# elybrand/quantized_neural_networks

Hardware: AMD Instinct MI355X
Metric: weights_quantized_per_sec (higher is better)
Workload: dtype f64; 1 GPU; Dense(4096->4096) whole-layer GPFQ, m=1024 calibration samples, M=3 alphabet, alphabet_scalar=3 (BASELINE.json configs[1], the north-star layer); N=4096, C=4096, m=1024, M=3, neurons_per_gpu=4096, arithmetic=f32 products / f64 residual and dot products (reference's mixed flow)

## Files before the change

quantized_neural_networks_amd/csrc/gpfq_blk.hip:

```cpp
#include <atomic>
#include <cmath>
#include <cstring>
#include <type_traits>

#include <cstdlib>
#include <mutex>
#include "gpfq_device.hpp"
#include <hip/hip_ext.h>
#include "gpfq_launch.hpp"
#include "gpfq_roles.hpp"

namespace gpfq {

namespace {

struct BlkStats {
    double rden, G, cb, ca, Ea, nrm;
    double sE1, sE2;
};
struct BandEntry {
    double H1, H2, E1, E2;
};
static_assert(sizeof(BlkStats) == 64 && sizeof(BandEntry) == 32, "header layout");

// ... 234 lines not shown
            for (int d = ND - 1; d >= 1; --d) { wx[d] = wx[d - 1]; wq[d] = wq[d - 1]; }
            wx[0] = xc; wq[0] = qc4;
            xc = xc1; qc4 = qc1; qn = qn1;
        }
    }
    __syncthreads();
    for (int w = threadIdx.x; w < RUN * (ND + 1); w += 256) {
        const int r = w / (ND + 1), e = w - r * (ND + 1);
        const int64_t t = t0 + r;
        if (t >= nrec) continue;
        auto total = [&](int k) { return (sm[r][0][k] + sm[r][1][k]) + (sm[r][2][k] + sm[r][3][k]); };
        char *rb = recs + t * rbytes;
        if (e == 0) {
            BlkStats st{};
            const double nrm = t < N ? (own_norms ? (double)(float)sqrt(nsm[r][0] + nsm[r][1] + nsm[r][2] + nsm[r][3]) : (double)nrm32[t]) : 0.0;
            const double s1 = total(1), s2 = total(2);
            st.nrm = nrm;
            st.rden = nrm < 1e-16 ? 0.0 : 1.0 / (nrm * nrm);
            st.G = total(0);
            st.cb = 0x1p-23 * s1 * st.rden * up;
            st.ca = 0x1p-149 * s2 * st.rden * up;
            st.Ea = 0x1p-149 * s2 * up;
            double e1 = 0.0, e2 = 0.0;
#pragma unroll
            for (int d = 1; d <= ND; ++d) { e1 += total(5 + 4 * (d - 1)); e2 += total(6 + 4 * (d - 1)); }
            st.sE1 = 0x1p-23 * e1 * up * up; st.sE2 = 0x1p-23 * e2 * up * up;
            *reinterpret_cast<BlkStats *>(rb) = st;
            *reinterpret_cast<BlkStats *>(hdrs + t * hdr) = st;
        } else {
            const int d = e;
            BandEntry be;
            be.H1 = total(3 + 4 * (d - 1)); be.H2 = total(4 + 4 * (d - 1));
            be.E1 = 0x1p-23 * total(5 + 4 * (d - 1)) * up; be.E2 = 0x1p-23 * total(6 + 4 * (d - 1)) * up;
            *reinterpret_cast<BandEntry *>(rb + 64 + 32 * (d - 1)) = be;
            *reinterpret_cast<BandEntry *>(hdrs + t * hdr + 64 + 32 * (d - 1)) = be;
        }
    }
}

__global__ void __launch_bounds__(256)
gpfq_blk_scale_kernel(char *__restrict__ recs, int64_t rec_bytes, int hdr, int mps, int64_t slice_bytes, const DevAlphabet *__restrict__ alpha)
{
    const float a = alpha->sym_a;
    float4 *row = reinterpret_cast<float4 *>(recs + (int64_t)blockIdx.y * slice_bytes + (int64_t)blockIdx.x * rec_bytes + hdr + 4 * (int64_t)mps);
    for (int i = threadIdx.x; i < mps / 4; i += 256) {
        const float4 v = row[i];
        row[i] = make_float4(__fmul_rn(a, v.x), __fmul_rn(a, v.y), __fmul_rn(a, v.z), __fmul_rn(a, v.w));
    }
}

template <int G, int NL, bool CL = false> constexpr bool blk_sweep_flush() { return (G == 4 && NL == 1) || CL; }

struct BlkLds {
    int tile_bytes, tile_pitch, off_w, off_d, off_wq, off_x2, off_e, off_out, off_ctl, off_zero, off_hr, hr_pitch, total;
};
constexpr int kOutSteps = 32;

__host__ __device__ constexpr int blk_sublanes(int nb) { return 64 / nb > 8 ? 8 : 64 / nb; }
__host__ __device__ constexpr int blk_slots(int nsw, int nb) { return (nsw + blk_sublanes(nb) - 1) / blk_sublanes(nb) * blk_sublanes(nb); }

__host__ __device__ inline BlkLds blk_lds(int mp, int nb, int B, int nsw, int G, bool CL = false)
{
    BlkLds L;
    const int nw = blk_slots(nsw, nb);
    L.tile_bytes = B * (int)blk_rec_bytes(mp, B, G, CL);
    L.tile_pitch = (L.tile_bytes + 1023) & ~1023;
    int o = 2 * L.tile_pitch;
    L.off_w = o;    o += 2 * nb * B * 4;    o = (o + 15) & ~15;
    L.off_d = o;    o += 2 * nw * B * nb * 8;
    L.off_wq = o;   o += 2 * nb * B * 8;
    L.off_x2 = o;   o += nw * nb * 16;
    L.off_e = o;    o += 68 * 8;
    L.off_out = o;  o += nb * kOutSteps * 8;
    L.off_ctl = o;  o += 16;
    L.off_zero = o; o += 32;
    o = (o + 15) & ~15;
    L.hr_pitch = (B * blk_hdr_bytes(B, CL) + 1023) & ~1023;
    L.off_hr = o;   o += 3 * L.hr_pitch;
    L.total = o;
    return L;
}

struct BlkK {
    const char *recs;
    const char *hdrs;
    const float *Wt;
    int64_t ldw, ldt;
    int64_t N, C;
    int m, M, zero_idx, nblk;
    int8_t *qidx;
    float *Qt;
    int64_t o_sj, o_st;
    const DevAlphabet *alpha;
    int *alpha_err;
    double *resid, *u_out;
    unsigned long long *fallback_count;
    unsigned long long *stamps;
    const float *Xq;
    int64_t ldx;
    unsigned char pw[12];
    int nsl;
    int cl_map;
    int64_t slice_bytes;
    unsigned long long *mbox;
    int64_t u_ld;
    double slack;
    int *cl_err;
    unsigned long long cl_timeout;
    int cl_fault;
};

#ifdef GPFQ_BLK_DIAG
#include "gpfq_blk_diag.hpp"
#else
constexpr bool kNoMfmaD = false, kNoFused = false;
#define STAMP(var) do { } while (0)
#define STAMP_DO(...)
#endif

struct ClState { int64_t cl; int slice; unsigned seq; bool dead; int64_t rec_off; int m_sl; };
typedef unsigned cl_u32x4 __attribute__((ext_vector_type(4)));

__device__ __forceinline__ cl_u32x4 cl_load16(const unsigned long long *p)
{
    cl_u32x4 r;
    asm volatile("global_load_dwordx4 %0, %1, off sc1" : "=&v"(r) : "v"(p) : "memory");
    return r;
}

template <int KV>
__device__ __forceinline__ void cl_publish(const BlkK &K, ClState &cs, int lane, const double (&v)[KV])
{
    const unsigned seq = ++cs.seq;
    if (K.cl_fault && cs.cl == 0 && cs.slice == 1) return;
    unsigned long long *buf = K.mbox + ((cs.cl * 2 + (int64_t)(seq & 1u)) * (int64_t)K.nsl) * 256;
    unsigned long long *mine = buf + ((int64_t)cs.slice * 64 + lane) * 4;
#pragma unroll
    for (int k = 0; k < KV; ++k) {
        const cl_u32x4 w = {(unsigned)__double2loint(v[k]), seq, (unsigned)__double2hiint(v[k]), seq};
        asm volatile("global_store_dwordx4 %0, %1, off sc1" :: "v"(mine + 2 * k), "v"(w) : "memory");
    }
}

template <int KV, int CLB>
__device__ __forceinline__ void cl_gather(const BlkK &K, ClState &cs, int lane, double (&v)[KV])
{
    const unsigned seq = cs.seq;
    const unsigned long long *buf = K.mbox + ((cs.cl * 2 + (int64_t)(seq & 1u)) * (int64_t)K.nsl) * 256;
    double tot[KV];
#pragma unroll
    for (int k = 0; k < KV; ++k) tot[k] = 0.0;
    const unsigned long long t0 = __builtin_amdgcn_s_memrealtime();
    for (int s0 = 0; s0 < K.nsl; s0 += CLB) {
        cl_u32x4 w[CLB][KV];
        for (;;) {
#pragma unroll
            for (int i = 0; i < CLB; ++i) {
                const unsigned long long *p = buf + ((int64_t)(s0 + i < K.nsl ? s0 + i : cs.slice) * 64 + lane) * 4;
#pragma unroll
                for (int k = 0; k < KV; ++k) w[i][k] = cl_load16(p + 2 * k);
            }
            asm volatile("s_waitcnt vmcnt(0)" ::: "memory");
// ... 166 lines not shown
        for (;;) {
            const int S = __builtin_amdgcn_readfirstlane(ctl);
            if (S < 0) break;
            const int nb_ = ((b + 1) & 1) * L.tile_pitch;
            const int cbq = (b & 1) * NB * B * 8;
            double eu[NL], ew[NL];
#pragma unroll
            for (int n = 0; n < NL; ++n) { eu[n] = 0.0; ew[n] = 0.0; }
#pragma unroll
            for (int n = 0; n < NL; ++n) {
                const float w = lds_ld<float2>(lds, o_wq + cbq + (n * B + S) * 8).x;
#pragma unroll 1
                for (int p = 0; p < PW; ++p) {
                    double t0 = u[n][0], t1 = u[n][1];
#pragma unroll
                    for (int pp = 1; pp < PW; ++pp) { t0 = (p == pp) ? u[n][2 * pp] : t0; t1 = (p == pp) ? u[n][2 * pp + 1] : t1; }
                    for (int j = 0; j < S; ++j) {
                        const int rb = nb_ + j * RB;
                        const float2 x2 = lds_ld<float2>(lds, rb + o_x + 8 * p * KQ), q2 = lds_ld<float2>(lds, rb + o_q + 8 * p * KQ);
                        const float2 wq = lds_ld<float2>(lds, o_wq + cbq + (n * B + j) * 8);
                        if constexpr (SYM) {
                            t0 += (double)__fmaf_rn(wq.y, q2.x, __fmul_rn(wq.x, x2.x));
                            t1 += (double)__fmaf_rn(wq.y, q2.y, __fmul_rn(wq.x, x2.y));
                        } else {
                            t0 += (double)__fsub_rn(__fmul_rn(wq.x, x2.x), __fmul_rn(wq.y, q2.x));
                            t1 += (double)__fsub_rn(__fmul_rn(wq.x, x2.y), __fmul_rn(wq.y, q2.y));
                        }
                    }
                    const int rb = nb_ + S * RB;
                    const float2 x2 = lds_ld<float2>(lds, rb + o_x + 8 * p * KQ);
                    float2 q2;
                    if constexpr (SYM) {
                        const int i0 = 2 * (pbase + p * KQ + kq);
                        const float *xr = K.Xq + ((int64_t)b * B + S) * K.ldx + (CL ? (int64_t)cs.slice * MP : (int64_t)0);
                        const int mrow = CL ? cs.m_sl : K.m;
                        q2.x = i0 < mrow ? xr[i0] : 0.f;
                        q2.y = i0 + 1 < mrow ? xr[i0 + 1] : 0.f;
                    } else {
                        q2 = lds_ld<float2>(lds, rb + o_q + 8 * p * KQ);
                    }
                    eu[n] = fma((double)q2.x, t0, eu[n]);
                    eu[n] = fma((double)q2.y, t1, eu[n]);
                    ew[n] = fma((double)q2.x, t0 + (double)__fmul_rn(w, x2.x), ew[n]);
                    ew[n] = fma((double)q2.y, t1 + (double)__fmul_rn(w, x2.y), ew[n]);
                }
            }
            const double vu = fold_klanes_n<G, NL>(eu), vw = fold_klanes_n<G, NL>(ew);
            if (writer) lds_st<double2>(lds, o_x2, make_double2(vu, vw));
            slot_barrier();
            slot_barrier();
            ctl = lds_ld<int>(lds, L.off_ctl + 4 * (b & 1));
        }
    };
    for (int b = 0; b < nslots; ++b) {
        STAMP(st0);
        STAMP_DO(if (b) acc_t += st0 - st5;)
        if (blk_sweep_flush<G, NL, CL>() && b >= 1 && wave == b % NSW && lane < NB * B && (!CL || cs.slice == 0)) {
            const int nn = lane / B, sidx = lane % B;
            const int64_t t = (int64_t)(b - 1) * B + sidx, jn = jbase + nn;
            if (t < N && jn < K.C) {
                const int2 v = lds_ld<int2>(lds, L.off_out + (nn * kOutSteps + (int)(t % kOutSteps)) * 8);
                if (K.qidx) K.qidx[jn * N + t] = (int8_t)v.x;
                if (K.Qt) K.Qt[jn * N + t] = __int_as_float(v.y);
            }
        }
        if (b + 1 < nslots) load_weights(b + 1);
        load_headers(b + 2, hbuf); hbuf = hbuf == 2 ? 0 : hbuf + 1;
        const int bn = b + 1 < nslots ? b + 1 : b;
        STAMP(st1);
        const int tbase = (b & 1) * L.tile_pitch;
        const int pbq = ((b - 1) & 1) * NB * B * 8;

        auto update_pair = [&](int p, const float2 &x2, const float2 &q2, const float (&wv)[NL], const float (&qv)[NL]) {
            const pk2 xv = {x2.x, x2.y}, qx = {q2.x, q2.y};
            pk2 pr[NL], rr[NL], dd[NL];
            double c0[NL], c1[NL];
#pragma unroll
            for (int n = 0; n < NL; ++n) pr[n] = pk2{wv[n], wv[n]} * xv;
            if constexpr (SYM) {
#pragma unroll
                for (int n = 0; n < NL; ++n) dd[n] = __builtin_elementwise_fma(pk2{qv[n], qv[n]}, qx, pr[n]);
            } else {
#pragma unroll
                for (int n = 0; n < NL; ++n) rr[n] = pk2{qv[n], qv[n]} * qx;
#pragma unroll
                for (int n = 0; n < NL; ++n) dd[n] = pr[n] - rr[n];
            }
#pragma unroll
            for (int n = 0; n < NL; ++n) { c0[n] = (double)dd[n].x; c1[n] = (double)dd[n].y; }
#pragma unroll
            for (int n = 0; n < NL; ++n) { u[n][2 * p] += c0[n]; u[n][2 * p + 1] += c1[n]; }
        };
        if constexpr (kFused) {
            const int rbm = tbase + ng * RB + o_d;
            constexpr int PF = NSW == 7 ? 2 : 1, NPS = PW * B;
            float2 fwq[B][NL], xbuf[PF], qbuf[PF];
            double2 dcur;
            auto row_off = [&](int i, bool q) { return tbase + (i % B) * RB + (q ? o_q : o_x) + 8 * (i / B) * KQ; };
            auto first_requests = [&]() {
#pragma unroll
                for (int s = 0; s < B; ++s)
#pragma unroll
                    for (int n = 0; n < NL; ++n) fwq[s][n] = lds_ld<float2>(lds, o_wq + pbq + (n * B + s) * 8);
#pragma unroll
                for (int i = 0; i < PF; ++i)
                    if (i < NPS) { xbuf[i] = lds_ld<float2>(lds, row_off(i, false)); qbuf[i] = lds_ld<float2>(lds, row_off(i, true)); }
                dcur = lds_ld<double2>(lds, rbm);
            };
            first_requests();
            double2 dprev = make_double2(0.0, 0.0);
            double acc[NL];
#pragma unroll
            for (int n = 0; n < NL; ++n) acc[n] = 0.0;
            auto mfma_pair = [&](int pp, int i, const double2 &dd) {
                const int n = i % NL, e = i / NL;
                acc[n] = __builtin_amdgcn_mfma_f64_4x4x4f64(u[n][2 * pp + e], e ? dd.y : dd.x, acc[n], 0, 0, 0);
            };
#pragma unroll
            for (int p = 0; p < PW; ++p) {
                {
                    const int pr = 2 - (3 * p) / PW;
                    if (p == 0 || pr != 2 - (3 * (p - 1)) / PW) {
                        const int v = pr;
                        if (v >= 2) __builtin_amdgcn_s_setprio(2);
                        else if (v == 1) __builtin_amdgcn_s_setprio(1);
                        else __builtin_amdgcn_s_setprio(0);
                    }
                }
                if (p > 0) dcur = lds_ld<double2>(lds, rbm + DB * p * KQ);
#pragma unroll
                for (int st = 0; st < B; ++st) {
                    const int ips = p * B + st;
                    const float2 x2 = xbuf[ips % PF], q2 = qbuf[ips % PF];
                    const int pn = (ips + 1) / B, sn = (ips + 1) % B;
                    (void)pn; (void)sn;
                    if (ips + PF < NPS) {
                        xbuf[ips % PF] = lds_ld<float2>(lds, row_off(ips + PF, false));
                        qbuf[ips % PF] = lds_ld<float2>(lds, row_off(ips + PF, true));
                    }
                    if (p < PTS) {
#pragma unroll
                        for (int i = 0; i < PPP; ++i) {
                            const int k = (PTS * st + p) * PPP + i;
                            if (PTS * B * PPP <= PER_MIN || k < PER_MIN) issue_piece(bn, k);
                        }
                    }
                    __builtin_amdgcn_sched_barrier(0);
                    float wv[NL], qv[NL];
#pragma unroll
                    for (int n = 0; n < NL; ++n) { wv[n] = fwq[st][n].x; qv[n] = fwq[st][n].y; }
                    update_pair(p, x2, q2, wv, qv);
                    if (p > 0) {
#pragma unroll
                        for (int i = 0; i < 2 * NL; ++i)
                            if (i * B / (2 * NL) == st) mfma_pair(p - 1, i, dprev);
                    }
                    __builtin_amdgcn_sched_barrier(0);
                }
                dprev = dcur;
            }
            for (int k = PTS * B * PPP < PER_MIN ? PTS * B * PPP : PER_MIN; wave + NSW * k < NPIECES; ++k) issue_piece(bn, k);
            STAMP(st2);
#pragma unroll
            for (int i = 0; i < 2 * NL; ++i) mfma_pair(PW - 1, i, dprev);
#pragma unroll
            for (int n = 0; n < NL; ++n) { acc[n] = ror_add<8>(acc[n]); acc[n] = ror_add<4>(acc[n]); }
            if (b + 1 < nslots && (lane & 12) == 0) {
                const int od = L.off_d + ((((((b + 1) & 1) * NW + wave) * B) + (lane & 3)) * NB + NL * (lane >> 4)) * 8;
                if constexpr (NL == 4) {
                    lds_st<double2>(lds, od, make_double2(acc[0], acc[1]));
                    lds_st<double2>(lds, od + 16, make_double2(acc[2], acc[3]));
                } else if constexpr (NL == 2) {
                    lds_st<double2>(lds, od, make_double2(acc[0], acc[NL - 1]));
                } else {
                    lds_st<double>(lds, od, acc[0]);
                }
            }
        } else {
        if constexpr (kPreloadAll) {
            if constexpr (!kHoist) { preload_wq(b); preload_rows(b); __builtin_amdgcn_sched_barrier(0); }
#pragma unroll
            for (int s = 0; s < B; ++s) {
                if (s == 0) __builtin_amdgcn_s_setprio(2);
                if (s == B / 2) __builtin_amdgcn_s_setprio(1);
                float wv[NL], qv[NL];
#pragma unroll
                for (int n = 0; n < NL; ++n) { wv[n] = wqa[s][n].x; qv[n] = wqa[s][n].y; }
#pragma unroll
                for (int p = 0; p < PW; ++p) {
                    if (p < PTS) {
#pragma unroll
// ... 78 lines not shown
                for (int p = 0; p < PW; ++p) {
                    if constexpr (kPreD) dsl[r][p] = ds[r][p];
                    else dsl[r][p] = ld_d(tbase + r * RB + o_d + DB * p * KQ);
                }
            if constexpr (!kPreD) __builtin_amdgcn_sched_barrier(0);
#pragma unroll
            for (int r = 0; r < B; ++r) {
                if (r == B / 2) __builtin_amdgcn_s_setprio(0);
                double acc[NL];
#pragma unroll
                for (int n = 0; n < NL; ++n) acc[n] = 0.0;
#pragma unroll
                for (int p = 0; p < PW; ++p) {
                    const double2 d2 = to_d2(dsl[r][p]);
#pragma unroll
                    for (int n = 0; n < NL; ++n) {
                        acc[n] = fma(d2.x, u[n][2 * p], acc[n]);
                        acc[n] = fma(d2.y, u[n][2 * p + 1], acc[n]);
                    }
                }
                const double v = fold_klanes_n<G, NL>(acc);
                if (writer) lds_st<double>(lds, o_dw + ((((b + 1) & 1) * NW) * B + r) * NB * 8, v);
            }
        } else
        if (b + 1 < nslots) {
            DRaw d2n = ld_d(tbase + o_d);
#pragma clang loop unroll_count(B == 4 ? 2 : 1)
            for (int r = 0; r < B; ++r) {
                if (r == B / 2) __builtin_amdgcn_s_setprio(0);
                double acc[NL];
#pragma unroll
                for (int n = 0; n < NL; ++n) acc[n] = 0.0;
                const int rb = tbase + r * RB;
                const int rn = r + 1 < B ? r + 1 : r;
#pragma unroll
                for (int p = 0; p < PW; ++p) {
                    const double2 d2 = to_d2(d2n);
                    const int rbn = p + 1 < PW ? rb : tbase + rn * RB, pn = p + 1 < PW ? p + 1 : 0;
                    d2n = ld_d(rbn + o_d + DB * pn * KQ);
                    __builtin_amdgcn_sched_barrier(0);
#pragma unroll
                    for (int n = 0; n < NL; ++n) {
                        acc[n] = fma(d2.x, u[n][2 * p], acc[n]);
                        acc[n] = fma(d2.y, u[n][2 * p + 1], acc[n]);
                    }
                    __builtin_amdgcn_sched_barrier(0);
                }
                const double v = fold_klanes_n<G, NL>(acc);
                if (writer) lds_st<double>(lds, o_dw + ((((b + 1) & 1) * NW) * B + r) * NB * 8, v);
            }
        }
        }
        STAMP(st3);
        dma_wait();
        STAMP(st4);
        slot_barrier();
        STAMP(st5);
        STAMP_DO(acc_dma += st1 - st0; acc_u += st2 - st1; acc_d += st3 - st2; acc_w += st4 - st3; acc_b += st5 - st4;)

        {
        int ctl = lds_ld<int>(lds, L.off_ctl + 4 * (b & 1));
        if constexpr (kHoist) {
            if (b + 1 < nslots) { preload_wq(b + 1); preload_rows(b + 1); }
        }
        if (__builtin_amdgcn_readfirstlane(ctl) >= 0) {
            slow_path(b, ctl);
            if constexpr (kHoist) {
                if (b + 1 < nslots) { preload_wq(b + 1); preload_rows(b + 1); }
            }
        }
        }
    }

    STAMP_DO(
    if (K.stamps && blockIdx.x == 0 && lane == 0 && (wave == 0 || wave == 7)) {
        unsigned long long *o = K.stamps + (wave == 0 ? 0 : 8);
        o[0] = acc_dma; o[1] = acc_u; o[2] = acc_d; o[3] = acc_w; o[4] = acc_b; o[5] = (unsigned long long)nslots; o[6] = acc_t;
    }
    if (K.stamps && blockIdx.x == 0 && lane == 0) K.stamps[32 + wave] = acc_dma + acc_u + acc_d + acc_w;

    )
    if (K.resid) {
        double ss[NL];
#pragma unroll
        for (int n = 0; n < NL; ++n) {
            double q = 0.0;
#pragma unroll
            for (int e = 0; e < 2 * PW; ++e) q = fma(u[n][e], u[n][e], q);
            ss[n] = q;
        }
        const double v = fold_klanes_n<G, NL>(ss);
        if (writer) lds_st<double>(lds, o_dw, v);
    }
    slot_barrier();
    if (K.u_out) {
#pragma unroll
        for (int n = 0; n < NL; ++n) {
            const int64_t jn = jbase + nloc + n;
            if (jn < K.C) {
#pragma unroll
                for (int p = 0; p < PW; ++p)
#pragma unroll
                    for (int e = 0; e < 2; ++e) {
                        const int i = 2 * (pbase + p * KQ + kq) + e;
                        if constexpr (CL) {
                            if (i < cs.m_sl) K.u_out[jn * K.u_ld + (int64_t)cs.slice * MP + i] = u[n][2 * p + e];
                        } else {
                            if (i < K.m) K.u_out[jn * (int64_t)K.m + i] = u[n][2 * p + e];
                        }
                    }
            }
        }
    }
}

template <int G, int MP, int B, int NSW, bool SYM, int NL, int CLM, bool KOUT = false>
__device__ __forceinline__ void blk_decision_role(const BlkK &K, char *lds_generic, const BlkLds &L, int lane, ClState &cs)
{
    constexpr bool CL = CLM != 0;
    constexpr int NB = NL * G, R = blk_sublanes(NB), NW = blk_slots(NSW, NB);
    constexpr int RB = (int)blk_rec_bytes(MP, B, G, CL);
    lchar *lds = (lchar *)lds_generic;
    const bool shadow = lane / R >= NB;
    const int n = shadow ? NB - 1 : lane / R, r = lane % R;
    const int64_t wg = cs.cl;
    const int64_t jn = wg * NB + n;
    const bool active = jn < K.C;
    const int64_t N = K.N;
    const int M = K.M;
    const int nslots = K.nblk + 1;
    const double kNaN = __longlong_as_double(0x7ff8000000000000LL);
    const int o_d   = L.off_d + (r * B * NB + n) * 8;
    const int o_x2  = L.off_x2 + (r * NB + n) * 16;
    const int o_w   = L.off_w + n * B * 4;
    const int o_wq  = L.off_wq + n * B * 8;
    const int o_out = L.off_out + n * kOutSteps * 8;

    const bool in_regs = M <= 4 * R;

    const double al_a0 = K.alpha->a0, al_step = K.alpha->step, al_inv = K.alpha->inv, al_c0 = K.alpha->c0;
    const unsigned long long al_plus = K.alpha->plus, al_minus = K.alpha->minus;
    const double sym_top = SYM ? lds_ld<double>(lds, L.off_e + 8 * (2 + M - 1)) : 0.0;
    const double sym_hb = (SYM && M == 3) ? 0.5 * sym_top : 0.0;
    float wprev[B], qprev[B];
    float wprev2[B], qprev2[B];
#pragma unroll
    for (int j = 0; j < B; ++j) { wprev[j] = 0.f; qprev[j] = 0.f; wprev2[j] = 0.f; qprev2[j] = 0.f; }
    double DmCur = 0.0;
    (void)wprev2; (void)qprev2; (void)DmCur;
    unsigned long long n_fallback = 0;
    auto wave_min_stop = [&](int v) -> int {
        int mn = B;
#pragma unroll
        for (int k = B - 1; k >= 0; --k)
            if (__ballot(v == k) != 0ull) mn = k;
        return mn;
    };

    constexpr bool kOwnFlush = !blk_sweep_flush<G, NL, CL>();
    auto flush = [&](int64_t t0, int64_t t1) {
        if constexpr (KOUT) {
            constexpr int NJ = NB < 8 ? NB : 8, GJ = NB / NJ;
            for (int e = lane; e < GJ * kOutSteps; e += 64) {
                const int g = e / kOutSteps, c = e % kOutSteps;
                const int64_t ts = t0 + c, j0 = wg * NB + g * NJ;
                if (ts >= t1 || j0 >= K.C || (CL && cs.slice != 0)) continue;
                int idxj[NJ]; float qj[NJ];
#pragma unroll
                for (int k = 0; k < NJ; ++k) {
                    const int2 v = lds_ld<int2>(lds, L.off_out + ((g * NJ + k) * kOutSteps + (int)(ts % kOutSteps)) * 8);
                    idxj[k] = v.x; qj[k] = __int_as_float(v.y);
                }
                const int64_t o = ts * K.o_st + j0;
                const bool whole = j0 + NJ <= K.C && K.o_sj == 1;
                if (K.qidx) {
                    if (whole && NJ >= 4 && ((uintptr_t)(K.qidx + o) & (NJ - 1)) == 0) {
                        unsigned lo = 0, hi = 0;
#pragma unroll
                        for (int k = 0; k < NJ; ++k) { if (k < 4) lo |= (unsigned)(idxj[k] & 0xff) << (8 * k); else hi |= (unsigned)(idxj[k] & 0xff) << (8 * (k - 4)); }
                        if constexpr (NJ == 8) *reinterpret_cast<uint2 *>(K.qidx + o) = make_uint2(lo, hi);
                        else *reinterpret_cast<unsigned *>(K.qidx + o) = lo;
                    } else {
#pragma unroll
                        for (int k = 0; k < NJ; ++k) if (j0 + k < K.C) K.qidx[ts * K.o_st + (j0 + k) * K.o_sj] = (int8_t)idxj[k];
                    }
                }
                if (K.Qt) {
                    if (whole && NJ >= 4 && ((uintptr_t)(K.Qt + o) & 15) == 0) {
#pragma unroll
                        for (int k = 0; k + 3 < NJ; k += 4) *reinterpret_cast<float4 *>(K.Qt + o + k) = make_float4(qj[k], qj[k + 1], qj[k + 2], qj[k + 3]);
                    } else {
#pragma unroll
                        for (int k = 0; k < NJ; ++k) if (j0 + k < K.C) K.Qt[ts * K.o_st + (j0 + k) * K.o_sj] = qj[k];
                    }
                }
            }
            return;
        }
        for (int e = lane; e < NB * (kOutSteps / 8); e += 64) {
            const int nn = e / (kOutSteps / 8), c = e % (kOutSteps / 8);
            const int64_t j = wg * NB + nn, ts = t0 + 8 * c;
            if (j >= K.C || ts >= t1 || (CL && cs.slice != 0)) continue;
            int idx8[8]; float q8[8];
// ... 240 lines not shown
            constexpr int NPEND = blk_band(B, CL);
            const double eps_q = fma((double)wmx, o67.x, u_amax * o67.y) + (double)NPEND * rEa;
            const bool sure_q = fabs(du_m) - eps_q >= 1e-10;
            const double delta2_q = base2 + 2.0 * eps_q * rden;
            const bool far_q = (d_lo - d_k > delta2_q) & (d_hi - d_k > delta2_q);
            ok = rule1 | (far_q & sure_q) | !valid_m;
            if (__ballot(!ok) != 0ull)
            {
                double2 ep[B], ei_[BI];
#pragma unroll
                for (int j = 0; j < B; ++j) ep[j] = lds_ld<double2>(lds, rbm + 64 + 32 * (B + sm - j - 1) + 16);
#pragma unroll
                for (int j = 0; j + 1 < B; ++j) ei_[j] = lds_ld<double2>(lds, j < sm ? rbm + 64 + 32 * (sm - j - 1) + 16 : L.off_zero);
#pragma unroll
                for (int j = 0; j < B; ++j) {
                    ePm = fma(fabs((double)wprev[j]), ep[j].x, ePm); ePm = fma(fabs((double)qprev[j]), ep[j].y, ePm);
                }
                if constexpr (CL) {
#pragma unroll
                    for (int j = 0; j < B; ++j) {
                        const double2 e2 = lds_ld<double2>(lds, rbm + 64 + 32 * (2 * B + sm - j - 1) + 16);
                        ePm = fma(fabs((double)wprev2[j]), e2.x, ePm); ePm = fma(fabs((double)qprev2[j]), e2.y, ePm);
                    }
                }
                double eps = ePm;
#pragma unroll
                for (int j = 0; j + 1 < B; ++j) { eps = fma(fabs(wd[j]), ei_[j].x, eps); eps = fma(fabs(qd[j]), ei_[j].y, eps); }
                unsigned any_m = anyP;
#pragma unroll
                for (int j = 0; j + 1 < B; ++j) any_m |= j < sm ? (__float_as_uint(wc[j]) | __float_as_uint(q32s[j])) : 0u;
                eps += ((any_m << 1) != 0u) ? (double)NPEND * rEa : 0.0;
                const bool du_exact = eps == 0.0;
                const bool msq = du_exact & small;
                const bool sure = du_exact | (fabs(du_m) - eps >= 1e-10);
                const double delta2 = base2 + 2.0 * eps * rden;
                const bool far = (d_lo - d_k > delta2) & (d_hi - d_k > delta2);
                const bool first = (d_k < d_lo) & (d_k <= d_hi);
                const bool cert = (msq ? first : far) & sure;
                ok = rule1 | cert | !valid_m;
            }
            const unsigned long long bad = __ballot(!ok);
            const float q_m = rule1 ? 0.f : qk32;
            const bool st = r < B;
            if (bad == 0ull) {
                STAMP(dtb);
#pragma unroll
                for (int s = 0; s < B; ++s) qc[s] = q32s[s];
                const float qpub = SYM ? (q_m > 0.f ? -1.f : (q_m < 0.f ? 1.f : 0.f)) : q_m;
                lds_st<float2>(lds, st ? o_wq + cbq + 8 * sm : o_dummy, make_float2(w_m, qpub));
                lds_st<int2>(lds, (st & valid_m) ? o_out + ((oslot0 + sm) % kOutSteps) * 8 : o_dummy,
                             make_int2(rule1 ? K.zero_idx : ki, __float_as_int(q_m)));
                ctl_now = -1;
                if (lane == 0) lds_st<int>(lds, L.off_ctl + 4 * (b & 1), -1);
            } else
            {
            const unsigned field = (unsigned)(bad >> (lane & ~(R - 1))) & ((1u << B) - 1u);
            stop = field ? __builtin_ctz(field) : B;
            STAMP(dtb);
#pragma unroll
            for (int s = 0; s < B; ++s) qc[s] = s < stop ? q32s[s] : 0.f;
            const bool keep = sm < stop;
            const float q_st = keep ? q_m : 0.f;
            const float qpub = SYM ? (q_st > 0.f ? -1.f : (q_st < 0.f ? 1.f : 0.f)) : q_st;
            lds_st<float2>(lds, st ? o_wq + cbq + 8 * sm : o_dummy, make_float2(w_m, qpub));
            lds_st<int2>(lds, (st & keep & valid_m) ? o_out + ((oslot0 + sm) % kOutSteps) * 8 : o_dummy,
                         make_int2(rule1 ? K.zero_idx : ki, __float_as_int(q_m)));
            const unsigned long long badA = __ballot(!ok & active);
            int smin = B;
#pragma unroll
            for (int k = B - 1; k >= 0; --k) {
                unsigned long long pat = 0ull;
#pragma unroll
                for (int g = 0; g < 64 / B; ++g) pat |= 1ull << (g * B + k);
                if (badA & pat) smin = k;
            }
            ctl_now = smin < B ? smin : -1;
            if (lane == 0) lds_st<int>(lds, L.off_ctl + 4 * (b & 1), ctl_now);
            }
            if constexpr (!kHdrChain) {
                asm volatile("s_waitcnt lgkmcnt(0)" ::: "memory");
                if constexpr (!CL) { if (b + 1 < K.nblk) prefetch_headers(hnext); }
            }
            if constexpr (CL) {
                if (b + 1 < K.nblk) {
                    double xv[1] = {0.0};
                    if (NL == 4 && K.nsl > 8) cl_gather<1, NL == 4 ? 16 : 8>(K, cs, lane, xv);
                    else cl_gather<1, 8>(K, cs, lane, xv);
                    DmCur = xv[0];
                }
            }
        } else {
            STAMP(dta);
            STAMP(dtb);
            if (lane == 0) lds_st<int>(lds, L.off_ctl + 4 * (b & 1), -1);
        }

        auto decide = [&](int s, bool commit, auto inregs_tag) -> bool {
            constexpr bool IN_REGS = decltype(inregs_tag)::value;
            double am[4];
#pragma unroll
            for (int q = 0; q < 4; ++q) am[q] = (IN_REGS && r + q * R < M) ? lds_ld<double>(lds, L.off_e + 8 * (2 + r + q * R)) : kNaN;
            const int rb = tbase + s * RB;
            const double2 r01 = lds_ld<double2>(lds, rb), r23 = lds_ld<double2>(lds, rb + 16), r45 = lds_ld<double2>(lds, rb + 32);
            const double rden = r01.x, rG = r01.y, rcb = r23.x, rca = r23.y, rEa = r45.x, nrm = r45.y;
            const bool rule1 = nrm < 1e-16;
            double corr = quad_bcast(cPm, s), eps = quad_bcast(ePm, s);
            unsigned anyinc = anyP;
#pragma unroll
            for (int j = 0; j < B; ++j) {
                if (j < s) {
                    const int d = s - j;
                    const double2 h = lds_ld<double2>(lds, rb + 64 + 32 * (d - 1)), e = lds_ld<double2>(lds, rb + 64 + 32 * (d - 1) + 16);
                    const double wj = (double)wc[j], qj = (double)qc[j];
                    corr = fma(wj, h.x, corr); corr = fma(-qj, h.y, corr);
                    eps = fma(fabs(wj), e.x, eps); eps = fma(fabs(qj), e.y, eps);
                    anyinc |= __float_as_uint(wc[j]) | __float_as_uint(qc[j]);
                }
            }
            eps += ((anyinc << 1) != 0u) ? (double)blk_band(B, CL) * rEa : 0.0;
            const double wd = (double)wc[s];
            const double du = D[s] + corr;
            const bool   du_exact = eps == 0.0;
            const bool   msq = du_exact & (fabs(du) < 1e-10);
            const bool   sure = du_exact | (fabs(du) - eps >= 1e-10);
            const double wG = wd * rG;
            const double tq = (du + wG) * rden;
            const double tt = msq ? wd : tq;
            const double delta2 = 2.0 * (fma(fabs(wd), rcb, rca) + eps * rden)
                                  + (CL ? K.slack : 0x1p-43) * (fabs(D[s]) + fabs(corr) + fabs(wG)) * rden;
            int idx_l;
// ... 63 lines not shown
#pragma unroll
                for (int q = 0; q < NW / R; ++q) d += lds_ld<double>(lds, o_d + ((((b & 1) * NW + q * R) * B) + s) * NB * 8);
                D[s] = sub_sum<R>(d);
            }
            }
            double du = 0.0, dw = 0.0;
#pragma unroll
            for (int q = 0; q < NW / R; ++q) {
                const double2 v = lds_ld<double2>(lds, o_x2 + q * R * NB * 16);
                du += v.x; dw += v.y;
            }
            du = sub_sum<R>(du); dw = sub_sum<R>(dw);
            if constexpr (CL) {
                double xv[2] = {du, dw};
                cl_exchange<2, 4>(K, cs, lane, xv);
                du = xv[0]; dw = xv[1];
            }
            const bool mine = active && stop == S;
            if (mine) {
                const int64_t t = (int64_t)b * B + S;
                const double nrm = lds_ld<double2>(lds, tbase + S * RB + 32).y;
                float wS = 0.f;
#pragma unroll
                for (int s = 0; s < B; ++s) wS = (s == S) ? wc[s] : wS;
                const double te = dw / (nrm * nrm);
                const double t2 = fabs(du) < 1e-10 ? (double)wS : te;
                int bi = 0;
                double bq = lds_ld<double>(lds, L.off_e + 16), bdist = fabs(bq - t2);
                for (int kk = 1; kk < M; ++kk) {
                    const double ak = lds_ld<double>(lds, L.off_e + 8 * (2 + kk)), dk = fabs(ak - t2);
                    if (dk < bdist) { bdist = dk; bi = kk; bq = ak; }
                }
                const float q32 = (float)bq;
#pragma unroll
                for (int s = 0; s < B; ++s) qc[s] = (s == S) ? q32 : qc[s];
                if (r == 0) {
                    lds_st<float2>(lds, o_wq + cbq + 8 * S, make_float2(wS, SYM ? (q32 > 0.f ? -1.f : (q32 < 0.f ? 1.f : 0.f)) : q32));
                    lds_st<int2>(lds, o_out + (int)(t % kOutSteps) * 8, make_int2(bi, __float_as_int(q32)));
                    if (!shadow) ++n_fallback;
                }
            }
            int stop2 = mine ? B : stop;
#pragma unroll
            for (int s = 0; s < B; ++s) {
                if (s > S) {
                    const bool ok = in_regs ? decide(s, mine && stop2 == B, T_{}) : decide(s, mine && stop2 == B, F_{});
                    if (mine && stop2 == B && !ok) stop2 = s;
                }
            }
            stop = stop2;
            const int smin = wave_min_stop(active ? stop : B);
            ctl_now = smin < B ? smin : -1;
            if (lane == 0) lds_st<int>(lds, L.off_ctl + 4 * (b & 1), ctl_now);
            slot_barrier();
        }

#pragma unroll
        for (int j = 0; j < B; ++j) {
            if constexpr (CL) { wprev2[j] = wprev[j]; qprev2[j] = qprev[j]; }
            wprev[j] = (b < K.nblk) ? wc[j] : 0.f; qprev[j] = (b < K.nblk) ? qc[j] : 0.f;
        }
        if constexpr (kOwnFlush) {
            const int64_t done = min((int64_t)(b + 1) * B, N);
            if (b < K.nblk && (done - flushed >= kOutSteps - B + 1 || done == N)) { flush_hi = done; }
        }
    }
    if constexpr (kOwnFlush) {
        if (flush_hi > flushed) { asm volatile("s_waitcnt lgkmcnt(0)" ::: "memory"); flush(flushed, flush_hi); }
    }

    if (K.fallback_count && n_fallback && (!CL || cs.slice == 0)) atomicAdd(K.fallback_count, n_fallback);
    STAMP_DO(if (K.stamps && blockIdx.x == 0 && lane == 0) { K.stamps[16] = dacc_work; K.stamps[17] = dacc_bar; K.stamps[18] = dacc_pro; K.stamps[19] = dacc_chain; K.stamps[20] = dacc_tail; })
    slot_barrier();
    if (K.resid) {
        double tot = 0.0;
#pragma unroll
        for (int q = 0; q < NW / R; ++q) tot += lds_ld<double>(lds, o_d + q * R * B * NB * 8);
        tot = sub_sum<R>(tot);
        if constexpr (CL) {
            double xv[1] = {tot};
            cl_exchange<1, 8>(K, cs, lane, xv);
            tot = xv[0];
        }
        if (active && r == 0 && (!CL || cs.slice == 0)) K.resid[jn] = sqrt(tot);
    }
}

}

template <int G, int S, int B, int NSW, bool SYM, int NL, int CLM = 0, bool KOUT = false>
__global__ void __launch_bounds__(64 * (NSW + 1))
gpfq_blk_kernel(BlkK K)
{
    constexpr bool CL = CLM != 0;
    constexpr int NB = NL * G, KQ = 64 / G, MP = 2 * KQ * S;
    if (K.alpha->ok == 0) {
        if (K.alpha_err && blockIdx.x == 0 && threadIdx.x == 0) *K.alpha_err = 1;
        return;
    }
    ClState cs{0, 0, 0u, false, 0, 0};
    if constexpr (CL) {
        const int id = (int)blockIdx.x, j = id >> 3;
        if (K.cl_map == 0) {
            cs.slice = j % K.nsl;
            cs.cl = (int64_t)(j / K.nsl) * 8 + (id & 7);
        } else {
// ... 146 lines not shown
    if (threadIdx.x != 0 || blockIdx.x != 0) return;
    form_device_alphabet(out, median32[0], alphabet_scalar, unit, want_sym);
}

static size_t blk_recs_bytes(int64_t nblk, const BlkShape &sh)
{
    return ((size_t)((nblk + 1) * sh.B + 1) * (size_t)blk_rec_bytes(sh.mp, sh.B, sh.G, sh.NS != 0) + 255) & ~(size_t)255;
}
static int64_t blk_clusters(int64_t C, const BlkShape &sh) { return (((C + sh.NL * sh.G - 1) / (sh.NL * sh.G)) + 7) / 8 * 8; }
static size_t blk_mbox_bytes(int64_t C, const BlkShape &sh) { return sh.NS > 1 ? (size_t)blk_clusters(C, sh) * 2 * sh.NS * 64 * 4 * 8 : 0; }
static size_t blk_hdrs_bytes(int64_t nblk, int B, bool CL = false) { return (size_t)((nblk + 1) * B + 1) * (size_t)blk_hdr_bytes(B, CL) + 2048; }
static size_t blk_hdrs_off(int64_t nblk, const BlkShape &sh) { return blk_recs_bytes(nblk, sh) * (size_t)(sh.NS ? sh.NS : 1); }
static size_t blk_mbox_off(int64_t nblk, const BlkShape &sh) { return blk_hdrs_off(nblk, sh) + ((blk_hdrs_bytes(nblk, sh.B, sh.NS != 0) + 255) & ~(size_t)255); }

bool blk_keras_out_supported(int64_t m, int64_t C, const Options &opt)
{
    const BlkShape sh = blk_shape(m, C, opt);
    return sh.G == 4 && sh.B == 4 && sh.NL == 4 && sh.NS == 0;
}

bool blk_supported(const PipeArgs &a)
{
    const BlkShape sh = blk_shape(a.m, a.C, a.opt);
    if (sh.G == 0 || a.N < 1 || a.m < 1) return false;
    if (a.A.M > 64 || !a.A.ascending) return false;
    DevAlphabet D{};
    D.M = a.A.M;
    for (int k = 0; k < a.A.M; ++k) D.a[k] = a.A.a[k];
    if (!blk_uniform(D)) return false;
    return a.N + 64 < (1LL << 31) / 64;
}

constexpr size_t kAlphaBlock = 1024;
static_assert(sizeof(DevAlphabet) <= kAlphaBlock, "alphabet block");

size_t blk_workspace_bytes(int64_t N, int64_t m, int64_t Cn, const Options &opt)
{
    if (m <= 0 || N < 0) return 0;
    size_t need = 0;
    for (int64_t C : {(int64_t)1 << 30, (int64_t)2048, (int64_t)1024, (int64_t)512, Cn > 0 ? Cn : (int64_t)1}) {
        const BlkShape sh = blk_shape(m, C, opt);
        if (!sh.G) continue;
        const int64_t nblk = (N + sh.B - 1) / sh.B;
        const size_t b = blk_recs_bytes(nblk, sh) * (size_t)(sh.NS ? sh.NS : 1) + ((blk_hdrs_bytes(nblk, sh.B, sh.NS != 0) + 255) & ~(size_t)255) + blk_mbox_bytes(Cn, sh);
        if (b > need) need = b;
    }
    return need ? need + kAlphaBlock : 0;
}

static float blk_sym_a(const PipeArgs &a)
{
    if ((a.opt.variant >> 4) & 2) return 0.f;
    return blk_sym_of(a.A.a, a.A.M);
}

constexpr bool blk_kout_shape(int G, int B, int NL, int CLM) { return G == 4 && B == 4 && NL == 4 && CLM == 0; }

template <int G, int S, int B, int NSW, bool SYM, int NL, int CLM = 0, bool KOUT = false>
static hipError_t launch_blk_sym(const PipeArgs &a, const BlkShape &sh, const DevAlphabet *alpha, hipStream_t stream)
{
    constexpr bool CL = CLM != 0;
    if constexpr (!KOUT && blk_kout_shape(G, B, NL, CLM)) {
        if (a.o_st != 1) return launch_blk_sym<G, S, B, NSW, SYM, NL, CLM, true>(a, sh, alpha, stream);
    }
    if (!KOUT && a.o_st != 1) return hipErrorInvalidValue;
    constexpr int NB = NL * G;
    const BlkLds L = blk_lds(sh.mp, NB, B, NSW, G, CL);
    const unsigned grid = CL ? (unsigned)(blk_clusters(a.C, sh) * sh.NS) : (unsigned)((a.C + NB - 1) / NB);
    auto *kern = gpfq_blk_kernel<G, S, B, NSW, SYM, NL, CLM, KOUT>;
    hipError_t e = ensure_dynamic_lds((const void *)kern, (size_t)L.total);
    if (e != hipSuccess) return e;
    BlkK K;
    const int64_t nblk_ = (a.N + B - 1) / B;
    char *const wbase = static_cast<char *>(a.workspace) + kAlphaBlock;
    K.recs = wbase; K.Wt = a.Wt; K.ldw = a.ldw; K.ldt = a.ldt;
    K.hdrs = K.recs + blk_hdrs_off(nblk_, sh);
    K.alpha = alpha;
    K.alpha_err = a.fallback_count ? reinterpret_cast<int *>(a.fallback_count + 1) + 1 : nullptr;
    K.nsl = CL ? sh.NS : 0; K.cl_map = blk_cluster_map(sh.NS, (a.C + NB - 1) / NB, a.opt); K.slice_bytes = (int64_t)blk_recs_bytes(nblk_, sh); K.mbox = nullptr; K.cl_err = nullptr;
    K.u_ld = a.m; K.slack = 0x1p-43 * (double)(sh.NS > 1 ? sh.NS : 1);
    K.cl_timeout = 100000ull * (unsigned long long)a.opt.blk_cluster_timeout_ms; K.cl_fault = a.opt.blk_cluster_fault;
    if constexpr (CLM == 1) {
        char *mb = wbase + blk_mbox_off(nblk_, sh);
        const size_t mbytes = blk_mbox_bytes(a.C, sh);
        e = hipMemsetAsync(mb, 0, mbytes, stream);
        if (e != hipSuccess) return e;
        K.mbox = reinterpret_cast<unsigned long long *>(mb);
        K.cl_err = a.fallback_count ? reinterpret_cast<int *>(a.fallback_count + 1) : nullptr;
    }
    K.N = a.N; K.C = a.C; K.m = (int)a.m; K.M = a.A.M; K.zero_idx = a.A.zero_idx; K.nblk = (int)((a.N + B - 1) / B);
    K.qidx = a.qidx; K.Qt = a.Qt; K.resid = a.resid; K.u_out = a.u_out; K.fallback_count = a.fallback_count;
    K.o_sj = a.o_st == 1 ? a.N : a.o_sj; K.o_st = a.o_st;
    K.stamps = a.fallback_count ? a.fallback_count + 8 : nullptr;
    K.Xq = a.Xq; K.ldx = a.ld;
    {
        const int *pw = blk_split<G, S, NSW, NL>();
        for (int w = 0; w < 12; ++w) K.pw[w] = (unsigned char)(w < NSW ? pw[w] : 0);
    }
    hipEvent_t ev0, ev1;
    if (main_kernel_events(&ev0, &ev1))
        hipExtLaunchKernelGGL(kern, dim3(grid), dim3(64 * (NSW + 1)), (unsigned)L.total, stream, ev0, ev1, 0, K);
    else
        hipLaunchKernelGGL(kern, dim3(grid), dim3(64 * (NSW + 1)), (size_t)L.total, stream, K);
    return hipGetLastError();
}

template <int G, int S, int B, int NSW = 8, int NL = 4>
static hipError_t launch_blk_inst(const PipeArgs &a, const BlkShape &sh, const DevAlphabet *alpha, hipStream_t stream)
{
    if (blk_sym_a(a) != 0.f) return launch_blk_sym<G, S, B, NSW, true, NL>(a, sh, alpha, stream);
    return launch_blk_sym<G, S, B, NSW, false, NL>(a, sh, alpha, stream);
}

struct ClusterLaunchGuard {
    static std::mutex &mu() { static std::mutex m; return m; }
    struct Last { hipEvent_t ev = nullptr; hipStream_t stream = nullptr; bool any = false; };
    static Last &last(int dev) { static Last L[64]; return L[dev & 63]; }
    std::unique_lock<std::mutex> lock;
    hipStream_t stream;
    int dev = 0;
    hipError_t err = hipSuccess;
    explicit ClusterLaunchGuard(hipStream_t s) : lock(mu()), stream(s)
    {
        err = hipGetDevice(&dev);
        if (err != hipSuccess) return;
        Last &l = last(dev);
        if (!l.ev) err = hipEventCreateWithFlags(&l.ev, hipEventDisableTiming);
        if (err == hipSuccess && l.any && l.stream != stream) err = hipStreamWaitEvent(stream, l.ev, 0);
    }
    ~ClusterLaunchGuard()
    {
        if (err != hipSuccess) return;
        Last &l = last(dev);
        if (hipEventRecord(l.ev, stream) == hipSuccess) { l.any = true; l.stream = stream; }
    }
};

static hipError_t blk_alphabet(const PipeArgs &a, const DevAlphabet **alpha, hipStream_t stream)
{
    if (a.dev_alpha) {
        *alpha = a.dev_alpha;
        return a.zero_counters && a.fallback_count ? hipMemsetAsync(a.fallback_count, 0, 64, stream) : hipSuccess;
    }
    DevAlphabet D{};
    D.M = a.A.M; D.zero_idx = a.A.zero_idx;
    D.rad = std::nan("");
    for (int k = 0; k < a.A.M && k < 64; ++k) D.a[k] = a.A.a[k];
// ... 159 lines not shown
```

quantized_neural_networks_amd/csrc/gpfq_roles.hpp:

```cpp
#pragma once

#include "gpfq_device.hpp"

namespace gpfq {
namespace {

constexpr int kSweepWaves = 8;

template <int ROR>
__device__ __forceinline__ double ror_add(double x)
{
    const int lo = __builtin_amdgcn_mov_dpp(__double2loint(x), 0x120 + ROR, 0xF, 0xF, true);
    const int hi = __builtin_amdgcn_mov_dpp(__double2hiint(x), 0x120 + ROR, 0xF, 0xF, true);
    return x + __hiloint2double(hi, lo);
}

__device__ __forceinline__ double fold32(double x, double y)
{
    const auto lo = __builtin_amdgcn_permlane32_swap((unsigned)__double2loint(x), (unsigned)__double2loint(y), false, false);
    const auto hi = __builtin_amdgcn_permlane32_swap((unsigned)__double2hiint(x), (unsigned)__double2hiint(y), false, false);
    return __hiloint2double((int)hi[0], (int)lo[0]) + __hiloint2double((int)hi[1], (int)lo[1]);
}

__device__ __forceinline__ double fold16(double x, double y)
// ... 74 lines not shown
{
    const double s02 = fold32(a[0], a[2]);
    const double s13 = fold32(a[1], a[3]);
    double x = fold16(s02, s13);
    if constexpr (G <= 8) x = ror_add<8>(x);
    if constexpr (G <= 4) x = ror_add<4>(x);
    if constexpr (G <= 2) x = ror_add<2>(x);
    if constexpr (G <= 1) x = ror_add<1>(x);
    return x;
}

template <int G, int NL>
__device__ __forceinline__ double fold_klanes_n(const double (&a)[NL])
{
    if constexpr (NL == 4) {
        return fold_klanes<G>(a);
    } else {
        double x = NL == 2 ? fold32(a[0], a[NL - 1]) : fold32(a[0], a[0]);
        x = fold16(x, x);
        if constexpr (G <= 8) x = ror_add<8>(x);
        if constexpr (G <= 4) x = ror_add<4>(x);
        if constexpr (G <= 2) x = ror_add<2>(x);
        if constexpr (G <= 1) x = ror_add<1>(x);
        return x;
    }
}

template <int CTRL>
__device__ __forceinline__ double dpp_add(double x)
{
    const int lo = __builtin_amdgcn_mov_dpp(__double2loint(x), CTRL, 0xF, 0xF, true);
    const int hi = __builtin_amdgcn_mov_dpp(__double2hiint(x), CTRL, 0xF, 0xF, true);
    return x + __hiloint2double(hi, lo);
}
template <int CTRL>
__device__ __forceinline__ int dpp_addi(int x) { return x + __builtin_amdgcn_mov_dpp(x, CTRL, 0xF, 0xF, true); }

template <int R> __device__ __forceinline__ double sub_sum(double x)
{
    if constexpr (R >= 2) x = dpp_add<0xB1>(x);
    if constexpr (R >= 4) x = dpp_add<0x4E>(x);
    if constexpr (R >= 8) x = dpp_add<0x141>(x);
    return x;
}
template <int R> __device__ __forceinline__ int sub_sumi(int x)
{
    if constexpr (R >= 2) x = dpp_addi<0xB1>(x);
    if constexpr (R >= 4) x = dpp_addi<0x4E>(x);
    if constexpr (R >= 8) x = dpp_addi<0x141>(x);
    return x;
}

__device__ __forceinline__ void slot_barrier() { asm volatile("s_waitcnt lgkmcnt(0)\n\ts_barrier" ::: "memory"); }

typedef float pk2 __attribute__((ext_vector_type(2)));

template <int S> struct PairSplit;
template <> struct PairSplit<32> { static constexpr int pw[8] = {2, 4, 4, 4, 3, 5, 5, 5}; };
template <> struct PairSplit<24> { static constexpr int pw[8] = {1, 3, 3, 3, 2, 4, 4, 4}; };
template <> struct PairSplit<16> { static constexpr int pw[8] = {1, 2, 2, 2, 1, 3, 3, 2}; };
template <> struct PairSplit<12> { static constexpr int pw[8] = {1, 2, 2, 1, 1, 2, 2, 1}; };
template <> struct PairSplit<8>  { static constexpr int pw[8] = {1, 1, 1, 1, 1, 1, 1, 1}; };
template <> struct PairSplit<40> { static constexpr int pw[8] = {5, 5, 5, 5, 5, 5, 5, 5}; };

typedef __attribute__((address_space(3))) char lchar;
typedef float  nf2 __attribute__((ext_vector_type(2)));
typedef float  nf4 __attribute__((ext_vector_type(4)));
typedef double nd2 __attribute__((ext_vector_type(2)));
typedef int    ni2 __attribute__((ext_vector_type(2)));
template <typename T> struct LdsNative { using type = T; };
template <> struct LdsNative<float2>  { using type = nf2; };
template <> struct LdsNative<float4>  { using type = nf4; };
template <> struct LdsNative<double2> { using type = nd2; };
template <> struct LdsNative<int2>    { using type = ni2; };
template <typename T> __device__ __forceinline__ T lds_ld(lchar *base, int off)
{
    using NT = typename LdsNative<T>::type;
    const NT v = *reinterpret_cast<__attribute__((address_space(3))) const NT *>(base + off);
    T out;
    __builtin_memcpy(&out, &v, sizeof(T));
    return out;
}
template <typename T> __device__ __forceinline__ void lds_st(lchar *base, int off, const T &v)
{
    using NT = typename LdsNative<T>::type;
    NT nv;
    __builtin_memcpy(&nv, &v, sizeof(T));
    *reinterpret_cast<__attribute__((address_space(3))) NT *>(base + off) = nv;
}

}
}
```

Baseline: 5.687 billion weights/s.

## Pre-read next slot's quantized weights and rows across the slot barrier

The decision wave now writes a sequence word to LDS alongside the control word. Sweep waves issue the LDS reads for the next slot's wq values, control and decision word before the barrier, and the row reads right after it. The barrier waits with a nonzero lgkmcnt so those reads stay in flight. If the decision word shows the next slot was decided on the fast path, the control reload and first-request reads are skipped. This aims to hide LDS latency at slot boundaries, at the cost of more register pressure and a fragile lgkmcnt accounting assumption.

```diff
diff --git a/quantized_neural_networks_amd/csrc/gpfq_blk.hip b/quantized_neural_networks_amd/csrc/gpfq_blk.hip
--- a/quantized_neural_networks_amd/csrc/gpfq_blk.hip
+++ b/quantized_neural_networks_amd/csrc/gpfq_blk.hip
@@ -310,7 +310,7 @@
 template <int G, int NL, bool CL = false> constexpr bool blk_sweep_flush() { return (G == 4 && NL == 1) || CL; }
 
 struct BlkLds {
-    int tile_bytes, tile_pitch, off_w, off_d, off_wq, off_x2, off_e, off_out, off_ctl, off_zero, off_hr, hr_pitch, total;
+    int tile_bytes, tile_pitch, off_w, off_d, off_wq, off_x2, off_e, off_out, off_ctl, off_dec, off_zero, off_hr, hr_pitch, total;
 };
 constexpr int kOutSteps = 32;
 
@@ -331,6 +331,7 @@
     L.off_e = o;    o += 68 * 8;
     L.off_out = o;  o += nb * kOutSteps * 8;
     L.off_ctl = o;  o += 16;
+    L.off_dec = o;  o += 16;
     L.off_zero = o; o += 32;
     o = (o + 15) & ~15;
     L.hr_pitch = (B * blk_hdr_bytes(B, CL) + 1023) & ~1023;
@@ -366,6 +367,7 @@
     int *cl_err;
     unsigned long long cl_timeout;
     int cl_fault;
+    int preread;
 };
 
 #ifdef GPFQ_BLK_DIAG
@@ -638,6 +640,30 @@
             ctl = lds_ld<int>(lds, L.off_ctl + 4 * (b & 1));
         }
     };
+    constexpr int PF = NSW == 7 ? 2 : 1, NPS = PW * B;
+    constexpr int FB = kFused ? B : 1, FN = kFused ? NL : 1;
+    float2 fwq[FB][FN], xbuf[PF], qbuf[PF];
+    double2 dcur = make_double2(0.0, 0.0);
+    auto row_off = [&](int tb, int i, bool q) { return tb + (i % B) * RB + (q ? o_q : o_x) + 8 * (i / B) * KQ; };
+    auto request_wq = [&](int b_) {
+        const int pbq_ = ((b_ - 1) & 1) * NB * B * 8;
+#pragma unroll
+        for (int s = 0; s < FB; ++s)
+#pragma unroll
+            for (int n = 0; n < FN; ++n) fwq[s][n] = lds_ld<float2>(lds, o_wq + pbq_ + (n * B + s) * 8);
+    };
+    auto request_rows = [&](int b_) {
+        const int tb = (b_ & 1) * L.tile_pitch;
+#pragma unroll
+        for (int i = 0; i < PF; ++i)
+            if (i < NPS) { xbuf[i] = lds_ld<float2>(lds, row_off(tb, i, false)); qbuf[i] = lds_ld<float2>(lds, row_off(tb, i, true)); }
+        dcur = lds_ld<double2>(lds, tb + ng * RB + o_d);
+    };
+    constexpr bool kPreRead = kFused && NL == 4 && PW <= 3;
+    const bool pre = kPreRead && K.preread != 0;
+    bool have_wq = false, have_rows = false;
+    (void)fwq; (void)xbuf; (void)qbuf; (void)dcur; (void)pre; (void)have_wq; (void)have_rows;
+    STAMP_DO(unsigned long long n_pre = 0, n_hit = 0;)
     for (int b = 0; b < nslots; ++b) {
         STAMP(st0);
         STAMP_DO(if (b) acc_t += st0 - st5;)
@@ -679,21 +705,8 @@
         };
         if constexpr (kFused) {
             const int rbm = tbase + ng * RB + o_d;
-            constexpr int PF = NSW == 7 ? 2 : 1, NPS = PW * B;
-            float2 fwq[B][NL], xbuf[PF], qbuf[PF];
-            double2 dcur;
-            auto row_off = [&](int i, bool q) { return tbase + (i % B) * RB + (q ? o_q : o_x) + 8 * (i / B) * KQ; };
-            auto first_requests = [&]() {
-#pragma unroll
-                for (int s = 0; s < B; ++s)
-#pragma unroll
-                    for (int n = 0; n < NL; ++n) fwq[s][n] = lds_ld<float2>(lds, o_wq + pbq + (n * B + s) * 8);
-#pragma unroll
-                for (int i = 0; i < PF; ++i)
-                    if (i < NPS) { xbuf[i] = lds_ld<float2>(lds, row_off(i, false)); qbuf[i] = lds_ld<float2>(lds, row_off(i, true)); }
-                dcur = lds_ld<double2>(lds, rbm);
-            };
-            first_requests();
+            if (!have_wq) request_wq(b);
+            if (!have_rows) request_rows(b);
             double2 dprev = make_double2(0.0, 0.0);
             double acc[NL];
 #pragma unroll
@@ -721,8 +734,8 @@
                     const int pn = (ips + 1) / B, sn = (ips + 1) % B;
                     (void)pn; (void)sn;
                     if (ips + PF < NPS) {
-                        xbuf[ips % PF] = lds_ld<float2>(lds, row_off(ips + PF, false));
-                        qbuf[ips % PF] = lds_ld<float2>(lds, row_off(ips + PF, true));
+                        xbuf[ips % PF] = lds_ld<float2>(lds, row_off(tbase, ips + PF, false));
+                        qbuf[ips % PF] = lds_ld<float2>(lds, row_off(tbase, ips + PF, true));
                     }
                     if (p < PTS) {
 #pragma unroll
@@ -907,19 +920,39 @@
         }
         }
         STAMP(st3);
-        dma_wait();
-        STAMP(st4);
-        slot_barrier();
+        int pre_dec = 0, pre_ctl = 0;
+        (void)pre_dec; (void)pre_ctl;
+        bool pre_now = false;
+        if constexpr (kPreRead) pre_now = pre && b + 1 < nslots;
+        if (pre_now) {
+            __builtin_amdgcn_sched_barrier(0);
+            pre_dec = lds_ld<int>(lds, L.off_dec);
+            pre_ctl = lds_ld<int>(lds, L.off_ctl + 4 * (b & 1));
+            request_wq(b + 1);
+            __builtin_amdgcn_sched_barrier(0);
+            dma_wait();
+            STAMP(st4);
+            slot_barrier_keep<2 * FN + 1>();
+            request_rows(b + 1);
+        } else {
+            dma_wait();
+            STAMP(st4);
+            slot_barrier();
+        }
         STAMP(st5);
         STAMP_DO(acc_dma += st1 - st0; acc_u += st2 - st1; acc_d += st3 - st2; acc_w += st4 - st3; acc_b += st5 - st4;)
-
-        {
+        have_wq = pre_now && __builtin_amdgcn_readfirstlane(pre_dec) == b + 1 && __builtin_amdgcn_readfirstlane(pre_ctl) < 0;
+        have_rows = pre_now;
+        STAMP_DO(n_pre += pre_now ? 1 : 0; n_hit += have_wq ? 1 : 0;)
+
+        if (!have_wq) {
         int ctl = lds_ld<int>(lds, L.off_ctl + 4 * (b & 1));
         if constexpr (kHoist) {
             if (b + 1 < nslots) { preload_wq(b + 1); preload_rows(b + 1); }
         }
         if (__builtin_amdgcn_readfirstlane(ctl) >= 0) {
             slow_path(b, ctl);
+            have_rows = false;
             if constexpr (kHoist) {
                 if (b + 1 < nslots) { preload_wq(b + 1); preload_rows(b + 1); }
             }
@@ -933,6 +966,7 @@
         o[0] = acc_dma; o[1] = acc_u; o[2] = acc_d; o[3] = acc_w; o[4] = acc_b; o[5] = (unsigned long long)nslots; o[6] = acc_t;
     }
     if (K.stamps && blockIdx.x == 0 && lane == 0) K.stamps[32 + wave] = acc_dma + acc_u + acc_d + acc_w;
+    if (K.stamps && blockIdx.x == 0 && lane == 0) K.stamps[21 + wave] = n_pre | (n_hit << 32);
 
     )
     if (K.resid) {
@@ -1004,6 +1038,7 @@
     double DmCur = 0.0;
     (void)wprev2; (void)qprev2; (void)DmCur;
     unsigned long long n_fallback = 0;
+    constexpr bool kDecWord = G == 4 && B == 4 && blk_row64(G, B) && !kNoMfmaD && !kNoFused;
     auto wave_min_stop = [&](int v) -> int {
         int mn = B;
 #pragma unroll
@@ -1350,6 +1385,7 @@
                              make_int2(rule1 ? K.zero_idx : ki, __float_as_int(q_m)));
                 ctl_now = -1;
                 if (lane == 0) lds_st<int>(lds, L.off_ctl + 4 * (b & 1), -1);
+                if (kDecWord && lane == 0) lds_st<int>(lds, L.off_dec, b + 1);
             } else
             {
             const unsigned field = (unsigned)(bad >> (lane & ~(R - 1))) & ((1u << B) - 1u);
@@ -1374,6 +1410,7 @@
             }
             ctl_now = smin < B ? smin : -1;
             if (lane == 0) lds_st<int>(lds, L.off_ctl + 4 * (b & 1), ctl_now);
+            if (kDecWord && lane == 0) lds_st<int>(lds, L.off_dec, b + 1);
             }
             if constexpr (!kHdrChain) {
                 asm volatile("s_waitcnt lgkmcnt(0)" ::: "memory");
@@ -1543,6 +1580,7 @@
             const int smin = wave_min_stop(active ? stop : B);
             ctl_now = smin < B ? smin : -1;
             if (lane == 0) lds_st<int>(lds, L.off_ctl + 4 * (b & 1), ctl_now);
+            if (kDecWord && lane == 0) lds_st<int>(lds, L.off_dec, b + 1);
             slot_barrier();
         }
 
@@ -1795,6 +1833,14 @@
 {
     if ((a.opt.variant >> 4) & 2) return 0.f;
     return blk_sym_of(a.A.a, a.A.M);
+}
+
+constexpr bool kPrereadDefault = true;
+static bool blk_preread(const Options &opt)
+{
+    if (opt.variant & 64) return false;
+    if (opt.variant & 128) return true;
+    return kPrereadDefault;
 }
 
 constexpr bool blk_kout_shape(int G, int B, int NL, int CLM) { return G == 4 && B == 4 && NL == 4 && CLM == 0; }
@@ -1836,6 +1882,7 @@
     K.o_sj = a.o_st == 1 ? a.N : a.o_sj; K.o_st = a.o_st;
     K.stamps = a.fallback_count ? a.fallback_count + 8 : nullptr;
     K.Xq = a.Xq; K.ldx = a.ld;
+    K.preread = blk_preread(a.opt) ? 1 : 0;
     {
         const int *pw = blk_split<G, S, NSW, NL>();
         for (int w = 0; w < 12; ++w) K.pw[w] = (unsigned char)(w < NSW ? pw[w] : 0);
diff --git a/quantized_neural_networks_amd/csrc/gpfq_roles.hpp b/quantized_neural_networks_amd/csrc/gpfq_roles.hpp
--- a/quantized_neural_networks_amd/csrc/gpfq_roles.hpp
+++ b/quantized_neural_networks_amd/csrc/gpfq_roles.hpp
@@ -150,6 +150,12 @@
 }
 
 __device__ __forceinline__ void slot_barrier() { asm volatile("s_waitcnt lgkmcnt(0)\n\ts_barrier" ::: "memory"); }
+template <int KEEP>
+__device__ __forceinline__ void slot_barrier_keep()
+{
+    static_assert(KEEP >= 0 && KEEP <= 15, "lgkmcnt is a four-bit counter");
+    asm volatile("s_waitcnt lgkmcnt(%0)\n\ts_barrier" :: "n"(KEEP) : "memory");
+}
 
 typedef float pk2 __attribute__((ext_vector_type(2)));
 
```

Result: no change. 5.734 billion weights/s, median of 6 (+0.8%).
